# vovach777/llcomp

Hardware: AMD Instinct MI355X
Metric: encode+decode MPix/s on 4K RGB8, bit-exact (higher is better)
Workload: dtype int32

## Files before the change

### llcomp_amd/csrc/geometry.hpp

```cpp
#pragma once
#include <algorithm>
#include <cstdint>
#include <cstdlib>

#if defined(__HIPCC__)
#define LLMI_HD __host__ __device__
#else
#define LLMI_HD
#endif

namespace llcomp_mi {

constexpr uint32_t kMaxChannels = 255;

struct Geometry {
    uint32_t frames, w, h, c;
    uint32_t tile_w, tile_h, planar;
    uint32_t ntx, nty;
    uint32_t slices_per_frame;
    uint32_t n_slices;
    uint32_t slice_cap;
    uint32_t nch;
    uint32_t lane_shift;
    uint32_t slice_samples;
    uint32_t lpw;
    uint32_t flags;
};
enum : uint32_t {
    kGeoRows = 1u,
    kGeoLdsTable = 2u,
    kGeoForceReplay = 4u,
    kGeoSmallModel = 8u,
    kGeoSnapshot = 16u,
    kGeoBankCache = 32u,
};
constexpr uint32_t kSnapMaxSamples = 4096;
constexpr uint32_t kSnapMaxChunks = 4;

struct Tuning {
    int lane_shift = -1;
    int lpw = 0;
    bool norows = false;
    bool noldstab = false;
    bool force_replay = false;
    bool nosnap = false;
    bool nocache = false;
    int overlap = 2;
    bool nofeedback = false;
};
inline Tuning tuning_from_env() {
    Tuning t;
    auto num = [](const char* name, long lo, long hi, int dflt) {
        const char* e = std::getenv(name);
        if (!e || !*e) return dflt;
        const long v = std::strtol(e, nullptr, 10);
        return (v >= lo && v <= hi) ? int(v) : dflt;
    };
    auto flag = [](const char* name) { const char* e = std::getenv(name); return e && e[0] == '1'; };
    t.lane_shift = num("LLCOMP_MI_LANE_SHIFT", 0, 6, -1);
    t.lpw = num("LLCOMP_MI_LPW", 1, 64, 0);
    t.norows = flag("LLCOMP_MI_NOROWS");
    t.noldstab = flag("LLCOMP_MI_NOLDSTAB");
    t.force_replay = flag("LLCOMP_MI_FORCE_REPLAY");
    t.nosnap = flag("LLCOMP_MI_NOSNAP");
    t.nocache = flag("LLCOMP_MI_NOCACHE");
    t.nofeedback = flag("LLCOMP_MI_NOFEEDBACK");
    t.overlap = num("LLCOMP_MI_OVERLAP", 0, 2, 2);
    return t;
}

LLMI_HD inline uint32_t snapshot_chunks(const Geometry& g) { return (g.slice_samples + kSnapMaxSamples - 1) / kSnapMaxSamples; }
LLMI_HD inline uint32_t snapshot_cap(const Geometry& g) {
    return g.slice_samples <= kSnapMaxSamples ? (g.slice_samples + 15u) & ~15u : snapshot_chunks(g) * kSnapMaxSamples;
}

constexpr int kBankCacheLog2 = 5;
inline int bank_cache_log2(const Geometry& g) { return (g.flags & kGeoBankCache) ? kBankCacheLog2 : 0; }

LLMI_HD inline uint32_t rows_px_dwords(uint64_t tile_base, uint32_t samples, uint32_t c, uint64_t batch_bytes) {
    if (tile_base + 4 > batch_bytes) return 0;
    const uint64_t k = (batch_bytes - 4 - tile_base) / c + 1;
    return k < samples ? uint32_t(k) : samples;
}
LLMI_HD inline uint32_t rows_px_tail(uint32_t c) { return 1 + (4 + c - 1) / c; }

LLMI_HD inline size_t lane_order_index(const Geometry& g, uint32_t id, uint32_t k) {
    const uint32_t gw = 1u << g.lane_shift;
    return ((size_t(id >> g.lane_shift) * g.slice_samples + k) << g.lane_shift) + (id & (gw - 1));
}

struct SliceRect {
    uint32_t frame, x0, y0, sw, sh, ch;
};

LLMI_HD inline SliceRect slice_rect(const Geometry& g, uint32_t id) {
    SliceRect r;
    r.frame = id / g.slices_per_frame;
    uint32_t s = id - r.frame * g.slices_per_frame;
    uint32_t tile = s;
    r.ch = 0;
    if (g.planar) {
        tile = s / g.c;
        r.ch = s - tile * g.c;
    }
    const uint32_t ty = tile / g.ntx, tx = tile - ty * g.ntx;
    r.x0 = tx * g.tile_w;
    r.y0 = ty * g.tile_h;
    r.sw = g.w - r.x0 < g.tile_w ? g.w - r.x0 : g.tile_w;
    r.sh = g.h - r.y0 < g.tile_h ? g.h - r.y0 : g.tile_h;
    return r;
}

inline uint32_t default_lane_shift(uint32_t n_slices) {
    constexpr uint32_t kMinWaves = 96;
    uint32_t s = 6;
    while (s > 0 && (n_slices >> s) < kMinWaves) --s;
    return s;
}

inline bool make_geometry(Geometry& g, uint32_t frames, uint32_t w, uint32_t h, uint32_t c, uint32_t tile_w,
                          uint32_t tile_h, uint32_t planar, const Tuning& tune = Tuning{}, bool small_model = false) {
    if (!frames || !w || !h || c < 1 || c > kMaxChannels) return false;
    if (tile_w == 0 || tile_w > w) tile_w = w;
    if (tile_h == 0 || tile_h > h) tile_h = h;
    const uint64_t samples = uint64_t(w) * h * c;
    if (samples >= (1ull << 31)) return false;
    g.frames = frames; g.w = w; g.h = h; g.c = c;
    g.tile_w = tile_w; g.tile_h = tile_h; g.planar = planar ? 1 : 0;
    g.ntx = (w + tile_w - 1) / tile_w;
    g.nty = (h + tile_h - 1) / tile_h;
    const uint64_t spf = uint64_t(g.ntx) * g.nty * (g.planar ? c : 1);
    if (spf * frames >= (1ull << 31)) return false;
    g.slices_per_frame = uint32_t(spf);
    g.n_slices = uint32_t(spf * frames);
    g.nch = g.planar ? 1 : c;
    const uint64_t cap = (uint64_t(tile_w) * tile_h * g.nch * 13 + 32 + 15) & ~15ull;
    g.slice_cap = uint32_t(cap < 0x7FFFFFF0ull ? cap : 0x7FFFFFF0ull);
    g.slice_samples = tile_w * tile_h * g.nch;
    g.lane_shift = tune.lane_shift >= 0 ? uint32_t(tune.lane_shift) : default_lane_shift(g.n_slices);
    if (tune.lane_shift < 0 && g.tile_h > 1 && g.slice_samples > kSnapMaxSamples && g.n_slices <= 512) g.lane_shift = 0;
    const uint32_t gw = 1u << g.lane_shift;
    g.lpw = gw;
    if (tune.lpw >= 1) {
        uint32_t p = 1;
        while (p * 2 <= uint32_t(tune.lpw) && p * 2 <= gw) p *= 2;
        g.lpw = p;
    }
    g.flags = 0;
    if (g.tile_h == 1 && !tune.norows && g.nch <= 4) g.flags |= kGeoRows;
    else if (g.lpw == 1 && !tune.noldstab) g.flags |= kGeoLdsTable;
    else if (g.slice_samples <= kSnapMaxSamples * kSnapMaxChunks && !tune.nosnap) g.flags |= kGeoSnapshot;
    if (!(g.flags & (kGeoRows | kGeoLdsTable)) && g.nch <= 4 && !tune.nocache) g.flags |= kGeoBankCache;
    if (tune.force_replay) g.flags |= kGeoForceReplay;
    if (small_model) g.flags |= kGeoSmallModel;
    return true;
}

inline uint64_t legacy_read_bound(uint64_t samples) { return 65 * samples + 2; }
inline void fit_legacy_stream(Geometry& g, uint64_t bytes) {
    const uint64_t cap = (bytes + 16 + 15) & ~15ull;
    if (cap > g.slice_cap) g.slice_cap = uint32_t(cap < 0x7FFFFFF0ull ? cap : 0x7FFFFFF0ull);
}

struct RegionBox {
    uint32_t tx0, ty0, tx1, ty1;
};
inline bool region_box(uint32_t w, uint32_t h, uint32_t tile_w, uint32_t tile_h, uint32_t x, uint32_t y, uint32_t rw, uint32_t rh,
                       RegionBox& b) {
    if (!w || !h || !rw || !rh || uint64_t(x) + rw > w || uint64_t(y) + rh > h) return false;
    if (tile_w == 0 || tile_w > w) tile_w = w;
    if (tile_h == 0 || tile_h > h) tile_h = h;
    const uint64_t ntx = (uint64_t(w) + tile_w - 1) / tile_w, nty = (uint64_t(h) + tile_h - 1) / tile_h;
    b.tx0 = x / tile_w;
    b.ty0 = y / tile_h;
    b.tx1 = uint32_t(std::min<uint64_t>((uint64_t(x) + rw + tile_w - 1) / tile_w, ntx));
    b.ty1 = uint32_t(std::min<uint64_t>((uint64_t(y) + rh + tile_h - 1) / tile_h, nty));
    return true;
}
inline bool region_geometry(const Geometry& full, const RegionBox& b, const Tuning& tune, Geometry& sub) {
    const uint32_t w = std::min<uint64_t>(uint64_t(b.tx1) * full.tile_w, full.w) - b.tx0 * full.tile_w;
    const uint32_t h = std::min<uint64_t>(uint64_t(b.ty1) * full.tile_h, full.h) - b.ty0 * full.tile_h;
    if (!make_geometry(sub, full.frames, w, h, full.c, full.tile_w, full.tile_h, full.planar, tune, (full.flags & kGeoSmallModel) != 0))
        return false;
    sub.slice_cap = full.slice_cap;
    return true;
}
LLMI_HD inline uint32_t region_full_id(const Geometry& full, const Geometry& sub, const RegionBox& b, uint32_t j) {
    const uint32_t f = j / sub.slices_per_frame, s = j - f * sub.slices_per_frame;
    const uint32_t planes = full.planar ? full.c : 1u;
    const uint32_t tile = s / planes, ch = s - tile * planes;
    const uint32_t ty = tile / sub.ntx, tx = tile - ty * sub.ntx;
    return f * full.slices_per_frame + ((b.ty0 + ty) * full.ntx + b.tx0 + tx) * planes + ch;
}
inline bool sub_arrays_fit(const Geometry& full, const Geometry& sub) {
    auto lanes = [](const Geometry& g) { return ((uint64_t(g.n_slices) + (1u << g.lane_shift) - 1) >> g.lane_shift) << g.lane_shift; };
    auto fused = [](const Geometry& g) { return g.planar && (g.flags & kGeoRows) && g.c <= 4; };
    if (sub.c != full.c || sub.n_slices > full.n_slices) return false;
    if (lanes(sub) > lanes(full)) return false;
    if (lanes(sub) * sub.slice_samples > lanes(full) * full.slice_samples) return false;
    if (uint64_t(lanes(sub)) * sub.slice_cap > uint64_t(lanes(full)) * full.slice_cap) return false;
    if (!fused(sub) && fused(full)) return false;
    return true;
}
inline bool region_fits(const Geometry& full, const Geometry& sub) { return sub.frames == full.frames && sub_arrays_fit(full, sub); }

LLMI_HD inline uint32_t region_sub_id(const Geometry& full, const Geometry& sub, const RegionBox& b, uint32_t id) {
    const uint32_t f = id / full.slices_per_frame, s = id - f * full.slices_per_frame;
    const uint32_t planes = full.planar ? full.c : 1u;
    const uint32_t tile = s / planes, ch = s - tile * planes;
    const uint32_t ty = tile / full.ntx, tx = tile - ty * full.ntx;
    if (tx < b.tx0 || tx >= b.tx1 || ty < b.ty0 || ty >= b.ty1) return ~0u;
    return f * sub.slices_per_frame + ((ty - b.ty0) * sub.ntx + tx - b.tx0) * planes + ch;
}
inline bool region_is_whole_box(const Geometry& full, const Geometry& sub, const RegionBox& b, uint32_t x, uint32_t y, uint32_t rw, uint32_t rh) {
    return x == b.tx0 * full.tile_w && y == b.ty0 * full.tile_h && rw == sub.w && rh == sub.h;
}
inline uint64_t snapshot_elems_of(const Geometry& g) {
    if (!(g.flags & kGeoSnapshot)) return 0;
    return (((uint64_t(g.n_slices) + (1u << g.lane_shift) - 1) >> g.lane_shift) * snapshot_cap(g)) << g.lane_shift;
}
inline uint64_t region_snapshot_bound(const Geometry& full) {
    if (full.flags & kGeoSnapshot) return snapshot_elems_of(full);
    if (full.flags & kGeoRows) return 0;
    if (!(full.flags & kGeoLdsTable) && full.slice_samples <= kSnapMaxSamples * kSnapMaxChunks) return 0;
    const uint64_t lanes = ((uint64_t(full.n_slices) + (1u << full.lane_shift) - 1) >> full.lane_shift) << full.lane_shift;
    const uint64_t cap = full.slice_samples <= kSnapMaxSamples ? (full.slice_samples + 15u) & ~15u
                                                               : uint64_t(std::min(snapshot_chunks(full), kSnapMaxChunks)) * kSnapMaxSamples;
    return lanes * cap;
}
inline bool region_encode_fits(const Geometry& full, const Geometry& sub) {
    if (!region_fits(full, sub)) return false;
    auto lanes = [](const Geometry& g) { return ((uint64_t(g.n_slices) + (1u << g.lane_shift) - 1) >> g.lane_shift) << g.lane_shift; };
    auto fused = [](const Geometry& g) { return g.planar && (g.flags & kGeoRows) && g.c <= 4; };
    auto lane_bytes = [&](const Geometry& g) { return std::max(lanes(g) * g.slice_samples * (fused(g) ? 2u : 4u), snapshot_elems_of(g) * 4); };
    if (lane_bytes(sub) > lane_bytes(full)) return false;
    if (snapshot_elems_of(sub) > region_snapshot_bound(full)) return false;
    if (lanes(sub) >> sub.lane_shift > uint64_t(full.n_slices)) return false;
// ... 57 lines not shown
```

### llcomp_amd/csrc/slice_kernels.hip

```cpp
#include <algorithm>

#include "device_common.hpp"
#include "kernels.hpp"

#ifndef LLMI_ASM_ENC
#define LLMI_ASM_ENC 1
#endif
#if LLMI_ASM_ENC
#include "enc_rows_asm.hpp"
#endif
#ifndef LLMI_ASM_DEC
#define LLMI_ASM_DEC 1
#endif
#if LLMI_ASM_DEC
#include "dec_rows_asm.hpp"
#endif

namespace llcomp_mi {

namespace {

#ifdef LLMI_CLOCK_PROBE
constexpr uint32_t kProbeSlots = 1u << 15;
__device__ unsigned long long g_probe[2][kProbeSlots][2];
struct ProbeStamp {
    unsigned long long t, r;
    __device__ __forceinline__ void start() {
        t = __builtin_amdgcn_s_memtime();
        r = __builtin_amdgcn_s_memrealtime();
    }
    __device__ __forceinline__ void stop(int kernel) {
        const unsigned long long t1 = __builtin_amdgcn_s_memtime(), r1 = __builtin_amdgcn_s_memrealtime();
        if (threadIdx.x == 0) {
            g_probe[kernel][blockIdx.x & (kProbeSlots - 1)][0] = t1 - t;
            g_probe[kernel][blockIdx.x & (kProbeSlots - 1)][1] = r1 - r;
        }
    }
};
#define LLMI_PROBE_START() ProbeStamp probe_stamp; probe_stamp.start()
#define LLMI_PROBE_STOP(kernel) probe_stamp.stop(kernel)
__device__ unsigned long long g_probe_parts[kProbeSlots][4];
struct PartClock {
    unsigned long long acc[4] = {0, 0, 0, 0}, last;
    __device__ __forceinline__ void start() { last = __builtin_amdgcn_s_memtime(); }
    __device__ __forceinline__ void lap(int part) {
        const unsigned long long now = __builtin_amdgcn_s_memtime();
        acc[part] += now - last;
        last = now;
    }
    __device__ __forceinline__ void flush() {
        if (threadIdx.x == 0)
            for (int k = 0; k < 4; ++k) g_probe_parts[blockIdx.x & (kProbeSlots - 1)][k] = acc[k];
    }
};
#define LLMI_PARTS_DECL() PartClock part_clock
#define LLMI_PARTS_START() part_clock.start()
#define LLMI_PARTS_LAP(part) part_clock.lap(part)
#define LLMI_PARTS_FLUSH() part_clock.flush()
#else
#define LLMI_PROBE_START() do {} while (0)
#define LLMI_PROBE_STOP(kernel) do {} while (0)
#define LLMI_PARTS_DECL() do {} while (0)
#define LLMI_PARTS_START() do {} while (0)
#define LLMI_PARTS_LAP(part) do {} while (0)
#define LLMI_PARTS_FLUSH() do {} while (0)
#endif

using entry_t = unsigned long long;
struct EntryTable {
    entry_t v[128];
};
constexpr EntryTable make_entries() {
    EntryTable t{};
    for (uint32_t s = 0; s < 128; ++s) t.v[s] = entry_t(entry_lo(s)) | (entry_t(entry_hi(s)) << 32);
    return t;
}
__constant__ EntryTable c_entries = make_entries();

using lds_u8_ptr = __attribute__((address_space(3))) uint8_t*;
using lds_entry_ptr = const __attribute__((address_space(3))) unsigned long long*;
__device__ __forceinline__ uint32_t lds_address(const void* p) { return uint32_t(uintptr_t((lds_u8_ptr) reinterpret_cast<const uint8_t*>(p))); }
__device__ __forceinline__ void load_table(entry_t* tab) {
    const unsigned long long rebase = (unsigned long long)lds_address(tab) * 0x0001000000010000ull;
    for (uint32_t i = threadIdx.x; i < 128; i += blockDim.x) tab[i] = c_entries.v[i] + rebase;
    __syncthreads();
}
__device__ __forceinline__ entry_t lds_entry(uint32_t address) { return *reinterpret_cast<lds_entry_ptr>(uintptr_t(address)); }

__device__ __forceinline__ void drain_vector_memory() { __builtin_amdgcn_s_waitcnt(0x0F70); }

__device__ __forceinline__ uint32_t byte_of(uint32_t w, int k) { return (w >> (8 * k)) & 0xFF; }
__device__ __forceinline__ uint32_t consume_here(uint32_t v);
template <int SLOT>
__device__ __forceinline__ uint32_t slot_state(const uint32_t* bank) {
    return byte_of(bank[SLOT >> 2], SLOT & 3);
}
template <int SLOT>
__device__ __forceinline__ void set_slot_state(uint32_t* bank, uint32_t ns) {
    constexpr int W = SLOT >> 2, SH = (SLOT & 3) * 8;
    bank[W] = (bank[W] & ~(0xFFu << SH)) | (ns << SH);
}
struct Bank {
    uint32_t w[4];
    uint8_t* lds;
};
constexpr uint32_t kRowBankWords = 3 * 2 * 64;
[[maybe_unused]] __device__ __forceinline__ constexpr uint32_t rowbank_byte(int slot) { return uint32_t(slot >> 2) * 256u + uint32_t(slot & 3); }
constexpr uint32_t kWideBankWords = 3 * 4 * 64;
__device__ __forceinline__ constexpr uint32_t widebank_byte(int slot) { return uint32_t(slot >> 1) * 256u + uint32_t(slot & 1) * 2u; }
template <int SLOT>
__device__ __forceinline__ uint32_t wide_offset(const uint32_t (&w)[4]) {
    return (SLOT & 1) ? (w[SLOT >> 1] >> 16) : (w[SLOT >> 1] & 0xFFFFu);
}
template <int SLOT, bool INLDS>
__device__ __forceinline__ void put_state(Bank& b, uint32_t ns) {
    if constexpr (INLDS) b.lds[rowbank_byte(SLOT)] = uint8_t(ns);
    else set_slot_state<SLOT>(b.w, ns & 0xFF);
}
__device__ __forceinline__ uint32_t prob_of(entry_t e) { return byte_of(uint32_t(e), 1); }
__device__ __forceinline__ uint32_t successor(entry_t e, bool bit) { return bit ? uint32_t(e >> 32) : uint32_t(e); }

struct Entries {
    entry_t e0, e1, e2, e3, e4, e5, e6, e7;
    template <int SLOT>
    __device__ __forceinline__ entry_t get() const {
        if constexpr (SLOT == 0) return e0;
        else if constexpr (SLOT == 1) return e1;
        else if constexpr (SLOT == 2) return e2;
        else if constexpr (SLOT == 3) return e3;
        else if constexpr (SLOT == 4) return e4;
        else if constexpr (SLOT == 5) return e5;
        else if constexpr (SLOT == 6) return e6;
        else return e7;
    }
};
__device__ __forceinline__ void fetch_slot0(Entries& E, const uint32_t* bank, const entry_t* tab) {
    E.e0 = tab[slot_state<0>(bank)];
}
__device__ __forceinline__ void fetch_rest(Entries& E, const uint32_t* bank, const entry_t* tab) {
    E.e1 = tab[slot_state<1>(bank)];
    E.e2 = tab[slot_state<2>(bank)];
    E.e3 = tab[slot_state<3>(bank)];
    E.e4 = tab[slot_state<4>(bank)];
    E.e5 = tab[slot_state<5>(bank)];
    E.e6 = tab[slot_state<6>(bank)];
    E.e7 = tab[slot_state<7>(bank)];
}

__device__ __forceinline__ entry_t entry_at(const entry_t*, uint32_t nx) { return lds_entry(nx >> 16); }

__device__ __forceinline__ void publish_count(unsigned long long* counters, uint32_t which, uint32_t mine) {
    if (!counters) return;
    unsigned long long live = __ballot(mine != 0);
// ... 36 lines not shown
    rest.x = a[4]; rest.y = a[5]; rest.z = a[6]; rest.w = a[7];
    if (e.flushed + 16 <= e.cap) *reinterpret_cast<uint4*>(e.gout + e.oofs) = v;
    e.oofs += e.ostep;
    a[0] = rest.x; a[1] = rest.y; a[2] = rest.z; a[3] = rest.w;
    e.flushed += 16;
    e.wp -= 16;
}
__device__ __forceinline__ void enc_carry_back(RangeEnc& e) {
    for (int32_t k = enc_pos(e) - 1; k >= 0; --k) {
        uint32_t v;
        if (k >= e.flushed) {
            uint8_t& r = e.area[k - e.flushed];
            v = r;
            r = uint8_t(v + 1);
        } else if (k < e.cap) {
            uint8_t* g = unit_byte(e, uint32_t(k));
            if (k == e.flushed - 1) ++e.carries;
            v = *g;
            *g = uint8_t(v + 1);
        } else {
            break;
        }
        if (v != 0xFF) break;
    }
}
__device__ __forceinline__ void enc_renorm(RangeEnc& e) {
    if (e.range < 0x100) {
        asm volatile("ds_write_b8_d16_hi %0, %1" : : "v"(e.wp), "v"(e.low) : "memory");
        const bool wrapped = e.low > 0xFFFFFFu;
        if (__builtin_expect(__builtin_amdgcn_ballot_w64(wrapped) != 0, 0)) {
            if (wrapped) enc_carry_back(e);
        }
        ++e.wp;
        asm("v_lshlrev_b32_sdwa %0, %1, %2 dst_sel:DWORD dst_unused:UNUSED_PAD src0_sel:DWORD src1_sel:WORD_0"
            : "=v"(e.low) : "v"(8u), "v"(e.low));
        e.range <<= 8;
    }
}
__device__ __forceinline__ void enc_core(RangeEnc& e, uint32_t P, uint32_t m) {
    const uint32_t r1 = __umul24(e.range, P) >> 8;
    const uint32_t r0 = e.range - r1;
    e.low += r0 & m;
    asm("v_bfi_b32 %0, %1, %2, %3" : "=v"(e.range) : "v"(m), "v"(r1), "v"(r0));
    enc_renorm(e);
}
__device__ __forceinline__ uint32_t successor_m(entry_t e, uint32_t m) {
    uint32_t r;
    asm("v_bfi_b32 %0, %1, %2, %3" : "=v"(r) : "v"(m), "v"(uint32_t(e >> 32)), "v"(uint32_t(e)));
    return r;
}
__device__ __forceinline__ uint32_t enc_step_msb(RangeEnc& e, uint32_t& bits, entry_t cur) {
    uint32_t off, r1;
    unsigned long long saved_exec;
    asm("v_add_co_u32_e32 %[bits], vcc, %[bits], %[bits]\n\t"
        "v_mul_u32_u24_sdwa %[r1], %[lo], %[range] dst_sel:DWORD dst_unused:UNUSED_PAD src0_sel:BYTE_1 src1_sel:DWORD\n\t"
        "v_lshrrev_b32_e32 %[r1], 8, %[r1]\n\t"
        "v_sub_u32_e32 %[range], %[range], %[r1]\n\t"
        "v_lshrrev_b32_e32 %[off], 16, %[lo]\n\t"
        "s_and_saveexec_b64 %[save], vcc\n\t"
        "v_add_u32_e32 %[low], %[low], %[range]\n\t"
        "v_mov_b32_e32 %[range], %[r1]\n\t"
        "v_lshrrev_b32_e32 %[off], 16, %[hi]\n\t"
        "s_mov_b64 exec, %[save]"
        : [bits] "+v"(bits), [range] "+v"(e.range), [low] "+v"(e.low), [off] "=&v"(off), [r1] "=&v"(r1), [save] "=&s"(saved_exec)
        : [lo] "v"(uint32_t(cur)), [hi] "v"(uint32_t(cur >> 32))
        : "vcc");
    enc_renorm(e);
    return off;
}
template <int SLOT, bool INLDS>
__device__ __forceinline__ void enc_once_m(RangeEnc& e, Bank& bank, const Entries& E, uint32_t m) {
    enc_core(e, prob_of(E.get<SLOT>()), m);
    put_state<SLOT, INLDS>(bank, successor_m(E.get<SLOT>(), m));
}
template <int SLOT, bool INLDS>
__device__ __forceinline__ void enc_once(RangeEnc& e, Bank& bank, const Entries& E, bool bit) {
    const entry_t en = E.get<SLOT>();
    const uint32_t r1 = __umul24(e.range, prob_of(en)) >> 8;
    if constexpr (INLDS) {
        e.range -= r1;
        put_state<SLOT, true>(bank, uint32_t(en));
        if (bit) {
            asm volatile("" : "+v"(e.low));
            e.low += e.range;
            e.range = r1;
            put_state<SLOT, true>(bank, uint32_t(en >> 32));
        }
        enc_renorm(e);
    } else {
        const uint32_t r0 = e.range - r1;
        e.low += bit ? r0 : 0u;
        e.range = bit ? r1 : r0;
        const uint32_t ns = successor(en, bit);
        enc_renorm(e);
        put_state<SLOT, INLDS>(bank, ns);
    }
}

template <bool ALL, bool INLDS>
__device__ __forceinline__ void enc_residual(RangeEnc& e, Bank& bank, const entry_t* tab, int res) {
    Entries E;
    fetch_slot0(E, bank.w, tab);
    if (ALL) fetch_rest(E, bank.w, tab);
    enc_once<0, INLDS>(e, bank, E, res == 0);
    if (res != 0) {
        if (!ALL) fetch_rest(E, bank.w, tab);
        const uint32_t a = uint32_t(res < 0 ? -res : res);
        const int ex = 31 - __clz(int(a));
        enc_once<1, INLDS>(e, bank, E, ex > 0);
        if (ex > 0) {
            enc_once<2, INLDS>(e, bank, E, ex > 1);
            if (ex > 1) {
                enc_once<3, INLDS>(e, bank, E, ex > 2);
                if (ex > 2) {
                    entry_t cur = E.e4;
                    const uint32_t ones = uint32_t(ex - 3);
                    uint32_t r1 = __umul24(e.range, prob_of(cur)) >> 8;
                    e.range -= r1;
                    for (uint32_t i = 0; i < ones; ++i) {
                        cur = entry_at(tab, uint32_t(cur >> 32));
                        e.low += e.range;
                        e.range = r1;
                        enc_renorm(e);
                        r1 = __umul24(e.range, prob_of(cur)) >> 8;
                        e.range -= r1;
                    }
                    enc_renorm(e);
                    put_state<4, INLDS>(bank, uint32_t(cur));
                }
            }
            enc_once_m<5, INLDS>(e, bank, E, uint32_t(__builtin_amdgcn_sbfe(int(a), uint32_t(ex - 1), 1u)));
            if (ex > 1) {
                entry_t cur = E.e6;
                uint32_t nx;
                uint32_t bits = ((a << 1) | 1u) << (32 - ex);
                do {
                    nx = enc_step_msb(e, bits, cur);
                    cur = lds_entry(nx);
                } while (bits != 0x80000000u);
                put_state<6, INLDS>(bank, (nx - lds_address(tab)) >> 3);
            }
        }
        enc_once<7, INLDS>(e, bank, E, res < 0);
    }
}

__device__ __forceinline__ void enc_finish_and_count(RangeEnc& e, int32_t& n_bytes) {
    e.range = 0xFF; e.low += 0xFF; enc_renorm(e);
    e.range = 0xFF; enc_renorm(e);
    n_bytes = enc_pos(e);
    while (int32_t(e.wp - e.base) > 0) enc_flush16(e);
}

extern __shared__ __attribute__((aligned(32))) unsigned char dyn_lds[];
constexpr uint32_t kRowsEncTabOff = 0, kRowsEncStageOff = 1024, kRowsEncBankOff = 1024 + 16 + 32 * 64;
constexpr uint32_t kRowsEncLdsBytes = kRowsEncBankOff + 3 * 64 * 8;
[[maybe_unused]] __device__ __forceinline__ void enc_carry_back_flushed(RangeEnc& e) {
    if (e.flushed > 0 && e.flushed - 1 < e.cap) ++e.carries;
    for (int32_t k = e.flushed - 1; k >= 0; --k) {
        if (k >= e.cap) break;
        uint8_t* g = unit_byte(e, uint32_t(k));
        const uint32_t v = *g;
        *g = uint8_t(v + 1);
        if (v != 0xFF) break;
    }
}
template <bool LDSTAB>
__device__ __forceinline__ void clear_lds_states() {
    if constexpr (LDSTAB) {
        unsigned long long* t = reinterpret_cast<unsigned long long*>(dyn_lds);
        for (uint32_t i = threadIdx.x; i < uint32_t(kContexts); i += blockDim.x) t[i] = 0;
    }
}
template <int NCH, bool ROWS, typename SYM, bool LDSTAB = false, bool SNAP = false, bool SEG = false>
__global__ __launch_bounds__(64) void k_encode_slices(const Geometry g, const uint32_t lpw,
                                                      const SYM* __restrict__ sym, uint64_t* __restrict__ states,
                                                      uint8_t* __restrict__ scratch, uint32_t* __restrict__ slice_len,
                                                      uint64_t* __restrict__ group_sum, uint32_t* status, const uint64_t gpat,
                                                      unsigned long long* __restrict__ counters, const uint32_t seg_first = 0,
                                                      uint32_t* __restrict__ seg_state = nullptr) {
    static_assert(!(SNAP && (ROWS || LDSTAB)) && (SNAP || !SEG), "one kernel family at a time");
    constexpr bool ASM = (ROWS || SNAP) && LLMI_ASM_ENC != 0;
    entry_t* tab;
    uint8_t* stage;
    uint32_t* rowbank;
    if constexpr (ASM) {
        static_assert(kStagePad == 16 && kStageBytes == 32, "kRowsEncBankOff");
#ifdef LLMI_TEST_LDS_OFFSET
        __shared__ uint32_t s_displace[4];
        if (threadIdx.x < 4) reinterpret_cast<volatile uint32_t*>(s_displace)[threadIdx.x] = gpat != 0;
#endif
        tab = reinterpret_cast<entry_t*>(dyn_lds + kRowsEncTabOff);
        stage = dyn_lds + kRowsEncStageOff;
        rowbank = reinterpret_cast<uint32_t*>(dyn_lds + kRowsEncBankOff);
        if (uint32_t(uintptr_t((lds_u8_ptr)dyn_lds)) != 0) {
            if (threadIdx.x == 0) atomicOr(status, kStInternal);
            return;
        }
    } else {
        __shared__ entry_t s_tab[128];
        __shared__ __attribute__((aligned(32))) uint8_t s_stage[kStagePad + kStageBytes * 64];
        __shared__ uint32_t s_rowbank[ROWS ? kRowBankWords : 1];
        tab = s_tab;
        stage = s_stage;
        rowbank = s_rowbank;
    }
    clear_lds_states<LDSTAB>();
    load_table(tab);
    const uint32_t id = blockIdx.x * lpw + threadIdx.x;
    if (threadIdx.x >= lpw || id >= g.n_slices) return;
    const SliceRect r = slice_rect(g, id);
    RangeEnc e;
    e.low = 0; e.range = 0xFF00;
    e.flushed = 0;
    e.area = stage + kStagePad + threadIdx.x * kStageBytes;
    e.base = uint32_t(uintptr_t((lds_u8_ptr)stage)) + kStagePad + threadIdx.x * kStageBytes;
    e.wp = e.base - 1;
    e.out = scratch + ((((size_t(id >> g.lane_shift) * (g.slice_cap >> 4)) << g.lane_shift) + (id & ((1u << g.lane_shift) - 1))) << 4);
    e.gout = scratch + (((size_t(__builtin_amdgcn_readfirstlane(id >> g.lane_shift)) * (g.slice_cap >> 4)) << g.lane_shift) << 4);
    e.oofs = (id & ((1u << g.lane_shift) - 1)) << 4;
    e.ostep = 16u << g.lane_shift;
    asm volatile("" : "+v"(e.ostep));
    e.cap = int32_t(g.slice_cap);
    e.shift = g.lane_shift;
    e.carries = 0;
    const uint32_t n_row = r.sw * (NCH ? uint32_t(NCH) : g.nch);
    const SYM* p0 = sym + lane_order_index(g, id, 0);
    const size_t GW = size_t(1) << g.lane_shift;
    const uint32_t total = n_row * r.sh;
    bool hot = false;
    LLMI_PROBE_START();

    if constexpr (SNAP) {
        const uint32_t cap = snapshot_cap(g);
        const uint32_t grp = __builtin_amdgcn_readfirstlane(id >> g.lane_shift);
        const char* const gres = reinterpret_cast<const char*>(sym) + ((size_t(grp) * cap * 2) << g.lane_shift);
        const char* const gbank = reinterpret_cast<const char*>(states) + ((size_t(grp) * cap * 8) << g.lane_shift);
        const uint32_t row = 32u << g.lane_shift;
        uint32_t lofs = (id & ((1u << g.lane_shift) - 1)) * 32u;
        asm volatile("" : "+v"(lofs));
        auto load_res = [&](uint32_t i) -> int {
            i = min(i, cap - 1);
            return *reinterpret_cast<const int16_t*>(gres + size_t(i >> 4) * row + ((i & 15u) << 1) + lofs);
        };
        auto load_bank = [&](uint32_t i) -> uint2 {
            i = min(i, cap - 1);
            return *reinterpret_cast<const uint2*>(gbank + size_t(i >> 3) * (2 * row) + ((i & 7u) << 3) + 2 * lofs);
        };
        uint32_t i = 0, end = total;
        [[maybe_unused]] uint32_t* const rec = SEG ? seg_state + size_t(id) * 16 : nullptr;
        if constexpr (SEG) {
            if (seg_first >= total) return;
            i = seg_first;
            end = min(total, seg_first + kSnapMaxSamples);
            if (seg_first) {
                const uint4 a = *reinterpret_cast<const uint4*>(rec), b = *reinterpret_cast<const uint4*>(rec + 4);
                const uint4 s0 = *reinterpret_cast<const uint4*>(rec + 8), s1 = *reinterpret_cast<const uint4*>(rec + 12);
                e.low = a.x; e.range = a.y; e.wp = e.base + a.z; e.flushed = int32_t(a.w);
                e.carries = b.x; hot = b.y != 0;
                e.oofs += (uint32_t(e.flushed) >> 4) * e.ostep;
                uint32_t* const st = reinterpret_cast<uint32_t*>(e.area);
                st[0] = s0.x; st[1] = s0.y; st[2] = s0.z; st[3] = s0.w; st[4] = s1.x; st[5] = s1.y; st[6] = s1.z; st[7] = s1.w;
            }
        }
#if LLMI_ASM_ENC
        EncRowsExtra xs{0u, 0u, 0u};
        unsigned long long low_range = e.low | ((unsigned long long)e.range << 32);
#endif
        auto code = [&](int res, uint2 bk) {
#if LLMI_ASM_ENC
            enc_snap_sample_asm(low_range, e.wp, xs, bk.x, bk.y, res, e.base);
            if (__builtin_expect(xs.any_pend != 0, 0)) {
                xs.any_pend = 0;
                if (xs.pend) enc_carry_back_flushed(e);
                xs.pend = 0;
            }
#else
            Bank bank{{bk.x, bk.y}, nullptr};
            if (hot) enc_residual<true, false>(e, bank, tab, res); else enc_residual<false, false>(e, bank, tab, res);
            hot = __builtin_amdgcn_readfirstlane(2 * __popcll(__ballot(res != 0)) >= __popcll(__ballot(true)));
#endif
        };
        const uint32_t todo = end - i, todo0 = __builtin_amdgcn_readfirstlane(todo);
        const bool same = __builtin_amdgcn_ballot_w64(todo != todo0) == 0;
        const uint32_t n_bulk = i + (same ? todo0 & ~3u : 0);
        int r0 = load_res(i), r1 = load_res(i + 1), r2 = load_res(i + 2), r3 = load_res(i + 3);
        uint2 b0 = load_bank(i), b1 = load_bank(i + 1), b2 = load_bank(i + 2), b3 = load_bank(i + 3);
#define LLMI_SNAP_SAMPLE(R, B, AHEAD)                          \
        {                                                          \
            const int rc = int(consume_here(uint32_t(R)));        \
            uint2 bc = B;                                          \
            bc.x = consume_here(bc.x);                             \
            R = load_res(i + AHEAD);                               \
            B = load_bank(i + AHEAD);                              \
            if (e.wp >= e.base + 16) enc_flush16(e);               \
            code(rc, bc);                                          \
        }
        for (; i < n_bulk; i += 4) {
            LLMI_SNAP_SAMPLE(r0, b0, 4)
            LLMI_SNAP_SAMPLE(r1, b1, 5)
            LLMI_SNAP_SAMPLE(r2, b2, 6)
            LLMI_SNAP_SAMPLE(r3, b3, 7)
        }
        for (; i < end; ++i) {
            LLMI_SNAP_SAMPLE(r0, b0, 4)
            {
                const int tr = r0;
                const uint2 tb = b0;
                r0 = r1; r1 = r2; r2 = r3; r3 = tr;
                b0 = b1; b1 = b2; b2 = b3; b3 = tb;
            }
        }
#undef LLMI_SNAP_SAMPLE
#if LLMI_ASM_ENC
        e.low = uint32_t(low_range);
        e.range = uint32_t(low_range >> 32);
#endif
        if constexpr (SEG) {
            if (end < total) {
                const uint32_t* const st = reinterpret_cast<const uint32_t*>(e.area);
                *reinterpret_cast<uint4*>(rec) = make_uint4(e.low, e.range, e.wp - e.base, uint32_t(e.flushed));
                *reinterpret_cast<uint4*>(rec + 4) = make_uint4(e.carries, hot ? 1u : 0u, 0u, 0u);
                *reinterpret_cast<uint4*>(rec + 8) = make_uint4(st[0], st[1], st[2], st[3]);
                *reinterpret_cast<uint4*>(rec + 12) = make_uint4(st[4], st[5], st[6], st[7]);
                return;
            }
        }
    } else if constexpr (ROWS) {
        for (uint32_t k = 0; k < 6; ++k) rowbank[k * 64 + threadIdx.x] = 0;
        constexpr bool PX = sizeof(SYM) == 1;
        const char* gsym;
        uint32_t sofs, sstep;
        [[maybe_unused]] uint32_t n_dword = total;
        [[maybe_unused]] uint32_t psh = 0, msub = 0, my = 0, large = 0;
        [[maybe_unused]] int pl = 128, pL = 128;
        if constexpr (PX) {
            const uint32_t C = g.c;
            const unsigned long long tbase = ((unsigned long long)(r.frame) * g.h + r.y0) * g.w * C + (unsigned long long)(r.x0) * C;
            const unsigned long long wbase = (unsigned long long)uint32_t(__builtin_amdgcn_readfirstlane(uint32_t(tbase))) |
                                             ((unsigned long long)uint32_t(__builtin_amdgcn_readfirstlane(uint32_t(tbase >> 32))) << 32);
            gsym = reinterpret_cast<const char*>(sym) + wbase;
            sofs = uint32_t(tbase - wbase);
            sstep = C;
            const unsigned long long total_bytes = (unsigned long long)(g.frames) * g.h * g.w * C;
            n_dword = rows_px_dwords(tbase, total, C, total_bytes);
            psh = 8 * r.ch;
            msub = C >= 3 && (r.ch == 0 || r.ch == 2) ? ~0u : 0u;
            my = C >= 3 && r.ch == 1 ? ~0u : 0u;
            large = (g.flags & kGeoSmallModel) ? 0u : ~0u;
            asm volatile("" : "+v"(psh), "+v"(msub), "+v"(my));
        } else {
            const uint32_t grp = __builtin_amdgcn_readfirstlane(id >> g.lane_shift);
            gsym = reinterpret_cast<const char*>(sym + ((size_t(grp) * g.slice_samples) << g.lane_shift));
            sofs = (id & ((1u << g.lane_shift) - 1)) * uint32_t(sizeof(SYM));
            sstep = uint32_t(sizeof(SYM)) << g.lane_shift;
        }
        asm volatile("" : "+v"(sstep));
        auto load_sym = [&](uint32_t ofs) -> uint32_t {
            if constexpr (PX) {
                uint32_t w;
                __builtin_memcpy(&w, gsym + ofs, 4);
                return w;
            } else {
                return *reinterpret_cast<const SYM*>(gsym + ofs);
            }
        };
        auto load_at = [&](uint32_t ofs, uint32_t k) -> uint32_t {
            if constexpr (PX) {
                if (k >= n_dword) {
                    const uint8_t* p = reinterpret_cast<const uint8_t*>(gsym + ofs);
                    uint32_t w = p[0];
                    if (g.c > 1) w |= uint32_t(p[1]) << 8;
                    if (g.c > 2) w |= uint32_t(p[2]) << 16;
                    if (g.c > 3) w |= uint32_t(p[3]) << 24;
                    return w;
                }
            }
            return load_sym(ofs);
        };
        uint32_t s0 = load_at(sofs, 0);
        sofs += sstep;
        uint32_t s1 = total > 1 ? load_at(sofs, 1) : 0;
        sofs += sstep;
        uint32_t bank_base = uint32_t(uintptr_t((lds_u8_ptr) reinterpret_cast<uint8_t*>(rowbank))) + threadIdx.x * 4;
        asm volatile("" : "+v"(bank_base));
#if LLMI_ASM_ENC
        EncRowsExtra xs{0u, 0u, 0u};
        unsigned long long low_range = e.low | ((unsigned long long)e.range << 32);
#endif
        auto code = [&](uint32_t sy, uint32_t i) {
            uint32_t bofs;
            int res;
            if constexpr (PX) {
                const uint32_t G = (sy >> 8) & 0xFF;
                const int sum = int(sy & 0xFF) + int((sy >> 16) & 0xFF) - 2 * int(G);
                const int t = (sum + int((uint32_t(sum) >> 31) * 3u)) >> 2;
                const int v = int(__builtin_amdgcn_ubfe(sy, psh, 8)) - int(G & msub) + (t & int(my));
                const int dq = (pL - pl) & int(i >= 2 ? large : 0u);
                const int sg = dq >> 31;
                const uint32_t aq = uint32_t((dq ^ sg) - sg);
                bofs = ((aq + 511u) & 0x200u) + ((aq + 508u) & 0x200u);
                res = ((v - pl) ^ sg) - sg;
                pL = pl;
                pl = v;
            } else if constexpr (sizeof(SYM) == 2) {
                bofs = (sy >> 3) & 0x600u;
                res = int(sy << 20) >> 20;
            } else {
                bofs = (((sy & 0xFFFF) * 109u) >> 7) & 0x600u;
                res = int(sy) >> 16;
            }
#if LLMI_ASM_ENC
            enc_rows_sample_asm(low_range, e.wp, xs, bank_base + bofs, res, e.base);
            if (__builtin_expect(xs.any_pend != 0, 0)) {
                xs.any_pend = 0;
                if (xs.pend) enc_carry_back_flushed(e);
                xs.pend = 0;
            }
#else
            uint32_t* bp = reinterpret_cast<uint32_t*>(reinterpret_cast<uint8_t*>(rowbank) + threadIdx.x * 4 + bofs);
            Bank bank{{bp[0], bp[64]}, reinterpret_cast<uint8_t*>(bp)};
            if (hot) enc_residual<true, true>(e, bank, tab, res); else enc_residual<false, true>(e, bank, tab, res);
            hot = __builtin_amdgcn_readfirstlane(2 * __popcll(__ballot(res != 0)) >= __popcll(__ballot(true)));
#endif
        };
        const uint32_t total0 = __builtin_amdgcn_readfirstlane(total);
        const bool same = __builtin_amdgcn_ballot_w64(total != total0) == 0;
        const uint32_t tail = PX ? rows_px_tail(g.c) : 2u;
        const uint32_t n_bulk = same && total0 > tail ? total0 - tail : 0;
        uint32_t i = 0;
        for (; i < n_bulk; ++i) {
            s0 = consume_here(s0);
            const uint32_t s2 = load_sym(sofs);
            sofs += sstep;
            if (e.wp >= e.base + 16) enc_flush16(e);
            code(s0, i);
            s0 = s1;
            s1 = s2;
        }
        for (; i < total; ++i) {
            s0 = consume_here(s0);
            const uint32_t s2 = i + 2 < total ? load_at(sofs, i + 2) : 0;
            sofs += sstep;
            if (e.wp >= e.base + 16) enc_flush16(e);
            code(s0, i);
            s0 = s1;
            s1 = s2;
        }
#if LLMI_ASM_ENC
        e.low = uint32_t(low_range);
        e.range = uint32_t(low_range >> 32);
#endif
    } else {
        uint64_t* banks;
        uint32_t bsh;
        if constexpr (LDSTAB) {
            banks = reinterpret_cast<uint64_t*>(dyn_lds);
            bsh = 0;
        } else {
            banks = states + ((size_t(id >> g.lane_shift) * kContexts) << g.lane_shift) + (id & ((1u << g.lane_shift) - 1));
            bsh = g.lane_shift;
        }
        uint32_t fk = 0;
        auto fetch = [&]() -> uint32_t { return p0[size_t(fk++) * GW]; };
        uint32_t s0 = fetch();
        uint32_t s1 = total > 1 ? fetch() : 0;
        uint64_t b0 = bank_fresh<LDSTAB>(banks[size_t(s0 & 0xFFFF) << bsh], gpat);
        for (uint32_t i = 0; i < total; ++i) {
            const uint32_t s2 = i + 2 < total ? fetch() : 0;
            const uint32_t ctx0 = s0 & 0xFFFF, ctx1 = s1 & 0xFFFF;
            const int res = int(s0) >> 16;
            uint64_t raw1 = (i + 1 < total) ? banks[size_t(ctx1) << bsh] : 0;
            Bank bank{{uint32_t(b0), uint32_t(b0 >> 32)}, nullptr};
            if (hot) enc_residual<true, false>(e, bank, tab, res); else enc_residual<false, false>(e, bank, tab, res);
            hot = __builtin_amdgcn_readfirstlane(2 * __popcll(__ballot(res != 0)) >= __popcll(__ballot(true)));
            b0 = uint64_t(bank.w[0]) | (uint64_t(bank.w[1]) << 32);
            if constexpr (!LDSTAB) drain_vector_memory();
            uint64_t b1 = bank_fresh<LDSTAB>(raw1, gpat);
            banks[size_t(ctx0) << bsh] = bank_tagged<LDSTAB>(b0, gpat);
            if (ctx1 == ctx0) b1 = b0;
            b0 = b1;
            if (e.wp >= e.base + 16) enc_flush16(e);
            s0 = s1;
            s1 = s2;
        }
    }
    int32_t n_bytes = enc_pos(e);
    enc_finish_and_count(e, n_bytes);
    LLMI_PROBE_STOP(0);
    if (n_bytes > e.cap) {
        atomicOr(status, kStOverflow);
        n_bytes = e.cap;
    }
    slice_len[id] = uint32_t(n_bytes);
    publish_count(counters, kCtrEncCarryBacks, e.carries);
    if (group_sum) {
        unsigned long long live = __ballot(1), sum = 0;
        while (live) {
            const int lane = __builtin_ctzll(live);
            sum += uint32_t(__builtin_amdgcn_readlane(n_bytes, lane));
            live &= live - 1;
        }
        if (threadIdx.x == 0) group_sum[blockIdx.x] = sum;
    }
}

template <int SLOT, bool INLDS>
__device__ __forceinline__ void dec_put_state(Bank& b, uint32_t half) {
    if constexpr (INLDS) *reinterpret_cast<uint16_t*>(b.lds + widebank_byte(SLOT)) = uint16_t(half >> 16);
    else set_slot_state<SLOT>(b.w, half & 0xFF);
}
template <int SLOT, bool INLDS>
__device__ __forceinline__ entry_t dec_entry(const Bank& b, const entry_t* tab) {
    if constexpr (INLDS) return lds_entry(wide_offset<SLOT>(b.w));
    else return tab[slot_state<SLOT>(b.w)];
}
template <bool INLDS>
__device__ __forceinline__ void dec_fetch_slot0(Entries& E, const Bank& b, const entry_t* tab) { E.e0 = dec_entry<0, INLDS>(b, tab); }
template <bool INLDS>
__device__ __forceinline__ void dec_fetch_rest(Entries& E, const Bank& b, const entry_t* tab) {
    E.e1 = dec_entry<1, INLDS>(b, tab);
    E.e2 = dec_entry<2, INLDS>(b, tab);
    E.e3 = dec_entry<3, INLDS>(b, tab);
    E.e4 = dec_entry<4, INLDS>(b, tab);
    E.e5 = dec_entry<5, INLDS>(b, tab);
    E.e6 = dec_entry<6, INLDS>(b, tab);
    E.e7 = dec_entry<7, INLDS>(b, tab);
}
struct RangeDec {
    uint32_t low, range;
    unsigned long long win;
    uint32_t nxt;
    const char* gbase;
    uint32_t ofs;
    uint32_t step;
    uint32_t ofs_end;
    uint32_t replays;
};
__device__ __forceinline__ bool window_low(const RangeDec& d) { return uint32_t(d.win >> 32) == 0; }
__device__ __forceinline__ void dec_prefetch(RangeDec& d) {
    d.nxt = *reinterpret_cast<const uint32_t*>(d.gbase + min(d.ofs, d.ofs_end));
    d.ofs += d.step;
}
__device__ __forceinline__ uint32_t consume_here(uint32_t v) {
    asm volatile("" : "+v"(v) : : "memory");
    return v;
}
__device__ __forceinline__ void dec_append(RangeDec& d) {
    const uint32_t ready = consume_here(d.nxt);
    const uint32_t sh = 31u - uint32_t(__builtin_clz(uint32_t(d.win)));
    const uint32_t rest = uint32_t(d.win) ^ (1u << sh);
    d.win = ((0x100000000ull | ready) << sh) | rest;
    dec_prefetch(d);
}
__device__ __forceinline__ void dec_append_drained(RangeDec& d) {
    dec_append(d);
    drain_vector_memory();
}
__device__ __forceinline__ void dec_open(RangeDec& d, const uint32_t* group, uint32_t lane, uint32_t shift, uint32_t len) {
    d.gbase = reinterpret_cast<const char*>(group);
    d.ofs = lane * 4;
    d.step = 4u << shift;
    asm volatile("" : "+v"(d.step));
    d.ofs_end = lane * 4 + ((len + 3) >> 2) * d.step;
    dec_prefetch(d);
    const uint32_t first = d.nxt;
    dec_prefetch(d);
    const unsigned long long both = first | ((unsigned long long)d.nxt << 32);
    dec_prefetch(d);
    d.range = 0xFF00;
    d.low = ((first & 0xFF) << 8) | ((first >> 8) & 0xFF);
    d.win = (both >> 16) | (1ull << 48);
    d.replays = 0;
}
__device__ __forceinline__ unsigned long long window_next(unsigned long long w) {
    unsigned long long r;
    asm("v_lshrrev_b64 %0, 8, %1" : "=v"(r) : "v"(w));
    return r;
}
__device__ __forceinline__ void dec_refill(RangeDec& d) {
    if (d.range < 0x100) {
        d.range <<= 8;
        d.low = (d.low << 8) | (uint32_t(d.win) & 0xFF);
        d.win = window_next(d.win);
    }
}
template <bool CHECKED>
__device__ __forceinline__ bool dec_core(RangeDec& d, uint32_t P) {
    if (CHECKED && d.win <= 1) dec_append_drained(d);
    const uint32_t r1 = __umul24(d.range, P) >> 8;
    const uint32_t r0 = d.range - r1;
    uint32_t diff;
    const bool under = __builtin_usub_overflow(d.low, r0, &diff);
    const bool bit = !under;
    d.low = under ? d.low : diff;
    d.range = under ? r0 : r1;
    dec_refill(d);
    return bit;
// ... 538 lines not shown
```

Measured before the change: 29290.

## Load packed pixels in four-pixel blocks in the rows encoder

Replaces the per-pixel unaligned dword load in the pixel-rows encode loop with one C-dword load per four pixels, templated on channel count. Each pixel is extracted from the block registers, and the next block is prefetched partway through coding the current one. The intent is fewer global load instructions and better latency hiding. The cost is more live registers, code duplicated per channel count, and a scalar tail loop for leftover pixels.

```diff
diff --git a/llcomp_amd/csrc/geometry.hpp b/llcomp_amd/csrc/geometry.hpp
--- a/llcomp_amd/csrc/geometry.hpp
+++ b/llcomp_amd/csrc/geometry.hpp
@@ -83,6 +83,19 @@
     return k < samples ? uint32_t(k) : samples;
 }
 LLMI_HD inline uint32_t rows_px_tail(uint32_t c) { return 1 + (4 + c - 1) / c; }
+
+constexpr uint32_t kRowsPxBlock = 4;
+LLMI_HD inline uint32_t rows_px_blocks(uint32_t samples) { return samples / kRowsPxBlock; }
+LLMI_HD inline uint32_t rows_px_block_bytes(uint32_t c) { return kRowsPxBlock * c; }
+LLMI_HD inline uint32_t rows_px_block_request(uint32_t b, uint32_t blocks) { return b + 1 < blocks ? b + 1 : blocks - 1; }
+template <int C, int J>
+LLMI_HD inline uint32_t rows_px_block_pixel(const uint32_t (&d)[C]) {
+    static_assert(C >= 1 && C <= 4 && J >= 0 && J < int(kRowsPxBlock), "1..4 channels, four pixels");
+    constexpr int at = J * C, lo = at / 4, sh = 8 * (at % 4);
+    if constexpr (sh == 0) return d[lo];
+    else if constexpr (sh + 8 * C <= 32) return d[lo] >> sh;
+    else return (d[lo] >> sh) | (d[lo + 1] << (32 - sh));
+}
 
 LLMI_HD inline size_t lane_order_index(const Geometry& g, uint32_t id, uint32_t k) {
     const uint32_t gw = 1u << g.lane_shift;
diff --git a/llcomp_amd/csrc/slice_kernels.hip b/llcomp_amd/csrc/slice_kernels.hip
--- a/llcomp_amd/csrc/slice_kernels.hip
+++ b/llcomp_amd/csrc/slice_kernels.hip
@@ -1,4 +1,5 @@
 #include <algorithm>
+#include <type_traits>
 
 #include "device_common.hpp"
 #include "kernels.hpp"
@@ -341,6 +342,26 @@
     while (int32_t(e.wp - e.base) > 0) enc_flush16(e);
 }
 
+#ifndef LLMI_ROWS_PX_BLOCK
+#define LLMI_ROWS_PX_BLOCK 1
+#endif
+template <int C>
+struct PxBlock {
+    uint32_t d[C];
+};
+template <int C>
+__device__ __forceinline__ PxBlock<C> px_block_load(const char* base, uint32_t ofs) {
+    PxBlock<C> b;
+    __builtin_memcpy(&b, base + ofs, sizeof(b));
+    return b;
+}
+template <int C>
+__device__ __forceinline__ void px_block_consume(PxBlock<C>& b) {
+    if constexpr (C == 1) asm volatile("" : "+v"(b.d[0]) : : "memory");
+    else if constexpr (C == 2) asm volatile("" : "+v"(b.d[0]), "+v"(b.d[1]) : : "memory");
+    else if constexpr (C == 3) asm volatile("" : "+v"(b.d[0]), "+v"(b.d[1]), "+v"(b.d[2]) : : "memory");
+    else asm volatile("" : "+v"(b.d[0]), "+v"(b.d[1]), "+v"(b.d[2]), "+v"(b.d[3]) : : "memory");
+}
 extern __shared__ __attribute__((aligned(32))) unsigned char dyn_lds[];
 constexpr uint32_t kRowsEncTabOff = 0, kRowsEncStageOff = 1024, kRowsEncBankOff = 1024 + 16 + 32 * 64;
 constexpr uint32_t kRowsEncLdsBytes = kRowsEncBankOff + 3 * 64 * 8;
@@ -518,6 +539,8 @@
     } else if constexpr (ROWS) {
         for (uint32_t k = 0; k < 6; ++k) rowbank[k * 64 + threadIdx.x] = 0;
         constexpr bool PX = sizeof(SYM) == 1;
+        constexpr bool PX_BLK = PX && LLMI_ROWS_PX_BLOCK != 0;
+        [[maybe_unused]] unsigned long long px_wbase = 0;
         const char* gsym;
         uint32_t sofs, sstep;
         [[maybe_unused]] uint32_t n_dword = total;
@@ -532,7 +555,8 @@
             sofs = uint32_t(tbase - wbase);
             sstep = C;
             const unsigned long long total_bytes = (unsigned long long)(g.frames) * g.h * g.w * C;
-            n_dword = rows_px_dwords(tbase, total, C, total_bytes);
+            if constexpr (!PX_BLK) n_dword = rows_px_dwords(tbase, total, C, total_bytes);
+            else px_wbase = wbase;
             psh = 8 * r.ch;
             msub = C >= 3 && (r.ch == 0 || r.ch == 2) ? ~0u : 0u;
             my = C >= 3 && r.ch == 1 ? ~0u : 0u;
@@ -544,7 +568,6 @@
             sofs = (id & ((1u << g.lane_shift) - 1)) * uint32_t(sizeof(SYM));
             sstep = uint32_t(sizeof(SYM)) << g.lane_shift;
         }
-        asm volatile("" : "+v"(sstep));
         auto load_sym = [&](uint32_t ofs) -> uint32_t {
             if constexpr (PX) {
                 uint32_t w;
@@ -567,17 +590,13 @@
             }
             return load_sym(ofs);
         };
-        uint32_t s0 = load_at(sofs, 0);
-        sofs += sstep;
-        uint32_t s1 = total > 1 ? load_at(sofs, 1) : 0;
-        sofs += sstep;
         uint32_t bank_base = uint32_t(uintptr_t((lds_u8_ptr) reinterpret_cast<uint8_t*>(rowbank))) + threadIdx.x * 4;
         asm volatile("" : "+v"(bank_base));
 #if LLMI_ASM_ENC
         EncRowsExtra xs{0u, 0u, 0u};
         unsigned long long low_range = e.low | ((unsigned long long)e.range << 32);
 #endif
-        auto code = [&](uint32_t sy, uint32_t i) {
+        auto code = [&](uint32_t sy, bool past2) {
             uint32_t bofs;
             int res;
             if constexpr (PX) {
@@ -585,7 +604,7 @@
                 const int sum = int(sy & 0xFF) + int((sy >> 16) & 0xFF) - 2 * int(G);
                 const int t = (sum + int((uint32_t(sum) >> 31) * 3u)) >> 2;
                 const int v = int(__builtin_amdgcn_ubfe(sy, psh, 8)) - int(G & msub) + (t & int(my));
-                const int dq = (pL - pl) & int(i >= 2 ? large : 0u);
+                const int dq = (pL - pl) & int(past2 ? large : 0u);
                 const int sg = dq >> 31;
                 const uint32_t aq = uint32_t((dq ^ sg) - sg);
                 bofs = ((aq + 511u) & 0x200u) + ((aq + 508u) & 0x200u);
@@ -616,14 +635,55 @@
         const uint32_t total0 = __builtin_amdgcn_readfirstlane(total);
         const bool same = __builtin_amdgcn_ballot_w64(total != total0) == 0;
         const uint32_t tail = PX ? rows_px_tail(g.c) : 2u;
-        const uint32_t n_bulk = same && total0 > tail ? total0 - tail : 0;
+        constexpr bool BLK = PX_BLK;
         uint32_t i = 0;
+        if constexpr (BLK) {
+            const uint32_t nblk = same ? rows_px_blocks(total0) : 0;
+            auto blocks = [&](auto cc) {
+                constexpr int CC = decltype(cc)::value;
+                constexpr uint32_t BB = kRowsPxBlock * CC;
+                PxBlock<CC> cur = px_block_load<CC>(gsym, sofs);
+                for (uint32_t b = 0; b < nblk; ++b) {
+                    px_block_consume(cur);
+#if LLMI_ASM_ENC
+                    xs.hot = __builtin_amdgcn_readfirstlane(xs.hot);
+#endif
+                    if (e.wp >= e.base + 16) enc_flush16(e);
+                    code(rows_px_block_pixel<CC, 0>(cur.d), b != 0);
+                    if (e.wp >= e.base + 16) enc_flush16(e);
+                    code(rows_px_block_pixel<CC, 1>(cur.d), b != 0);
+                    const uint32_t p2 = rows_px_block_pixel<CC, 2>(cur.d), p3 = rows_px_block_pixel<CC, 3>(cur.d);
+                    if (e.wp >= e.base + 16) enc_flush16(e);
+                    code(p2, true);
+                    cur = px_block_load<CC>(gsym, sofs + rows_px_block_request(b, nblk) * BB);
+                    if (e.wp >= e.base + 16) enc_flush16(e);
+                    code(p3, true);
+                }
+            };
+            if (nblk) {
+                switch (g.c) {
+                    case 1: blocks(std::integral_constant<int, 1>{}); break;
+                    case 2: blocks(std::integral_constant<int, 2>{}); break;
+                    case 3: blocks(std::integral_constant<int, 3>{}); break;
+                    default: blocks(std::integral_constant<int, 4>{}); break;
+                }
+                i = nblk * kRowsPxBlock;
+                sofs += nblk * rows_px_block_bytes(g.c);
+            }
+            n_dword = i + rows_px_dwords(px_wbase + sofs, total - i, g.c, (unsigned long long)(g.frames) * g.h * g.w * g.c);
+        }
+        asm volatile("" : "+v"(sstep));
+        uint32_t s0 = !BLK || i < total ? load_at(sofs, i) : 0;
+        sofs += sstep;
+        uint32_t s1 = i + 1 < total ? load_at(sofs, i + 1) : 0;
+        sofs += sstep;
+        const uint32_t n_bulk = !BLK && same && total0 > tail ? total0 - tail : 0;
         for (; i < n_bulk; ++i) {
             s0 = consume_here(s0);
             const uint32_t s2 = load_sym(sofs);
             sofs += sstep;
             if (e.wp >= e.base + 16) enc_flush16(e);
-            code(s0, i);
+            code(s0, i >= 2);
             s0 = s1;
             s1 = s2;
         }
@@ -632,7 +692,7 @@
             const uint32_t s2 = i + 2 < total ? load_at(sofs, i + 2) : 0;
             sofs += sstep;
             if (e.wp >= e.base + 16) enc_flush16(e);
-            code(s0, i);
+            code(s0, i >= 2);
             s0 = s1;
             s1 = s2;
         }
```

Result: no change. 29620, median of 6 (+1.1%).
